# senikm/trpx

Measured on AMD Instinct MI355X. Metric: frames/s (Terse encode + Prolix decode round trip, 512x512 uint16 stack, bit-exact vs CPU ref), higher is better.
Workload: dtype u16

## Files before the change

__graft_entry__.py:

```python
import os
import subprocess
import sys

ROOT = os.path.dirname(os.path.abspath(__file__))
if ROOT not in sys.path:
    sys.path.insert(0, ROOT)


def build() -> None:
    jobs = str(min(8, os.cpu_count() or 1))
    subprocess.check_call(["make", "-s", "-j", jobs, "-C", os.path.join(ROOT, "trpx_amd", "csrc")])
    subprocess.check_call(["make", "-s", "-C", os.path.join(ROOT, "trpx_amd", "csrc"), "force_timeout", "weakparts", "chain_timeout", "denseserial", "densetiny", "segfbgrid", "segwgrounds", "alldense", "noclassify"])
    subprocess.check_call(["make", "-s", "-C", os.path.join(ROOT, "oracle"), "all"])
    if os.path.isdir("/root/reference/include"):
        subprocess.check_call(["make", "-s", "-C", os.path.join(ROOT, "oracle"), "ref"])
    subprocess.check_call(["make", "-s", "-C", os.path.join(ROOT, "trpx_amd", "cli")])
    subprocess.check_call(["make", "-s", "-C", os.path.join(ROOT, "tests", "cpp")])
    subprocess.check_call(["make", "-s", "-C", os.path.join(ROOT, "tests", "cpp"), "-f", "roi_example.mk"])
    subprocess.check_call(["make", "-s", "-C", os.path.join(ROOT, "tests", "cpp"), "-f", "encode_sparse_example.mk"])
    subprocess.check_call(["make", "-s", "-C", os.path.join(ROOT, "tests", "cpp"), "-f", "decode_plan_test.mk"])
    subprocess.check_call([os.path.join(ROOT, "tests", "cpp", "encode_sparse_sanitize")], stdout=subprocess.DEVNULL)
    import tempfile
    with tempfile.TemporaryDirectory() as d:
        subprocess.check_call([os.path.join(ROOT, "tests", "cpp", "host_sanitize"), os.path.join(d, "t.trpx")], stdout=subprocess.DEVNULL)
    import trpx_amd
    from trpx_amd import _lib
    _lib.lib()
# ... 35 lines not shown
```

trpx_amd/csrc/encode_fused.hip:

```cpp
#include <stddef.h>
#include <utility>
#include "codec_common.hpp"
#include "launchers.hpp"
#include "profile.hpp"
#include <stdlib.h>
#include <mutex>
#include <vector>

namespace trpx {

#ifndef TRPX_FUSED_SUB32
#define TRPX_FUSED_SUB32 5
#endif
#ifndef TRPX_FUSED_SUB16
#define TRPX_FUSED_SUB16 4
#endif
template <typename T> constexpr int sub_tiles() { return sizeof(T) <= 2 ? TRPX_FUSED_SUB16 : TRPX_FUSED_SUB32; }
#ifndef TRPX_FUSED_OCC16
#define TRPX_FUSED_OCC16 8
#endif
#ifndef TRPX_FUSED_OCC32
#define TRPX_FUSED_OCC32 4
#endif
template <typename T> constexpr int fused_occupancy() { return sizeof(T) == 1 ? 8 : (sizeof(T) == 2 ? TRPX_FUSED_OCC16 : TRPX_FUSED_OCC32); }
// ... 70 lines not shown
    }
    *result = acc;
    return true;
}

constexpr int kAccShift = 40;
#ifndef TRPX_FUSED_ACC_LINES
#define TRPX_FUSED_ACC_LINES 2
#endif
constexpr uint32_t kAccLines = TRPX_FUSED_ACC_LINES;
__host__ __device__ inline uint32_t fused_acc_lines(uint32_t tiles_per_frame) {
    const uint32_t k = (tiles_per_frame + 31u) / 32u;
    return k < 1u ? 1u : (k > kAccLines ? kAccLines : k);
}
constexpr uint64_t kPrefFlag = 1ull << 63;
__device__ bool lookback_frames(const uint64_t* __restrict__ acc_w, const uint64_t* __restrict__ pref_w, int64_t frame,
                                uint64_t tiles_per_frame, uint64_t* result, uint64_t stride, uint32_t n_acc) {
    const int lane = lane_id();
    uint64_t acc = 0;
    int64_t pos = frame - 1;
    while (pos >= 0) {
        const int64_t my = pos - lane;
        const bool in = my >= 0;
        uint64_t p = in ? 0ull : kPrefFlag, c = 0;
        uint32_t first_p = 64;
        SpinGuard guard;
        uint64_t need = ~0ull;
        bool complete = false;
        for (;;) {
            if (in && !(p & kPrefFlag) && !complete && ((need >> lane) & 1ull)) {
// ... 21 lines not shown
}

template <typename T> struct Raw {
    static constexpr int bits = PixelTraits<T>::bits;
    static constexpr int per = 32 / bits;
    static constexpr int dw = kBlock / per;
};

template <typename T>
__device__ __forceinline__ uint32_t raw_field(const uint32_t (&raw)[Raw<T>::dw], int k) {
    constexpr int per = Raw<T>::per, bits = Raw<T>::bits;
    const uint32_t x = raw[k / per] >> ((k % per) * bits);
    return bits == 32 ? x : x & ((1u << (bits & 31)) - 1u);
}

template <typename T> struct QuadVec;
template <> struct QuadVec<uint8_t>  { typedef uint32_t type; };
template <> struct QuadVec<int8_t>   { typedef uint32_t type; };
template <> struct QuadVec<uint16_t> { typedef uint32_t type __attribute__((ext_vector_type(2))); };
template <> struct QuadVec<int16_t>  { typedef uint32_t type __attribute__((ext_vector_type(2))); };
template <> struct QuadVec<uint32_t> { typedef uint32_t type __attribute__((ext_vector_type(4))); };
template <> struct QuadVec<int32_t>  { typedef uint32_t type __attribute__((ext_vector_type(4))); };

template <typename T>
__device__ __forceinline__ void load_raw_nt(const T* __restrict__ p, uint32_t (&raw)[Raw<T>::dw]) {
    if constexpr (sizeof(T) == 2) {
        typedef uint32_t u4 __attribute__((ext_vector_type(4)));
        typedef uint32_t u2 __attribute__((ext_vector_type(2)));
        u4 lo; u2 hi;
        __builtin_memcpy(&lo, p, 16);
// ... 28 lines not shown
    __builtin_memcpy(&lo, q, 16);
    __builtin_memcpy(&hi, q + 16, 8);
    __builtin_memcpy(&last, q + 24, 2);
    raw[0] = __builtin_amdgcn_alignbit(lo.y, lo.x, 16); raw[1] = __builtin_amdgcn_alignbit(lo.z, lo.y, 16);
    raw[2] = __builtin_amdgcn_alignbit(lo.w, lo.z, 16); raw[3] = __builtin_amdgcn_alignbit(hi.x, lo.w, 16);
    raw[4] = __builtin_amdgcn_alignbit(hi.y, hi.x, 16); raw[5] = __builtin_amdgcn_alignbit((uint32_t)last, hi.y, 16);
}
template <typename T>
__device__ __forceinline__ void load_raw_partial(const T* __restrict__ p, int nb, uint32_t (&raw)[Raw<T>::dw]) {
    using UT = typename PixelTraits<T>::U;
#pragma unroll
    for (int i = 0; i < Raw<T>::dw; ++i) raw[i] = 0;
#pragma unroll
    for (int k = 0; k < kBlock; ++k)
        if (k < nb) raw[k / Raw<T>::per] |= (uint32_t)(UT)p[k] << ((k % Raw<T>::per) * Raw<T>::bits);
}

template <typename T>
__device__ __forceinline__ uint32_t raw_width(const uint32_t (&raw)[Raw<T>::dw]) {
    constexpr int bits = Raw<T>::bits;
    uint32_t m = 0;
    if (!PixelTraits<T>::is_signed) {
#pragma unroll
        for (int i = 0; i < Raw<T>::dw; ++i) m |= raw[i];
        if (bits == 16) m = (m | (m >> 16)) & 0xFFFFu;
        if (bits == 8) { m |= m >> 16; m = (m | (m >> 8)) & 0xFFu; }
    } else if (bits == 32) {
#pragma unroll
        for (int i = 0; i < Raw<T>::dw; ++i) {
            const uint32_t u = raw[i];
// ... 135 lines not shown
    uint64_t* bnd_pos;
    uint64_t* frame_acc;
    uint64_t* frame_pref;
    uint64_t* frame_base;
    uint32_t acc_stride;
    uint32_t n_acc;
    uint64_t* ws_tag;
    uint64_t expect_tag;
    uint64_t* frame_offsets;
    uint32_t* out32;
    uint32_t* status;
    uint8_t* idx_widths;
    uint64_t* idx_group_off;
    uint32_t debug;
    uint64_t* stamps;
};

typedef const char __attribute__((address_space(4)))* karg_ptr;
#define TRPX_KARG(kb, field) (*reinterpret_cast<const decltype(FusedArgs::field) __attribute__((address_space(4)))*>((kb) + 8 + offsetof(FusedArgs, field)))

template <typename T, bool MIS2>
__device__ __forceinline__ void encode_fused_body(const T* __restrict__ pixels, const FusedArgs& a) {
    constexpr int kSub = sub_tiles<T>();
    constexpr int kFusedTileBlocks = kSub * kThreads;
    constexpr int kStage = fused_stage_dwords<T>();
    constexpr int kStage4 = (kStage + 1 + 3) / 4;
    __shared__ __attribute__((aligned(16))) uint32_t s_stage_pad[4 * kStage4];
    uint32_t* const s_stage = s_stage_pad + 1;
    __shared__ uint32_t s_hdr[40];
    __shared__ uint32_t s_wtot[kSub * 4];
    __shared__ uint32_t s_wfl[kSub * 4];
    __shared__ uint64_t s_excl_bits;
    __shared__ uint64_t s_base_bytes;
    __shared__ uint32_t s_abort;
    __shared__ uint32_t s_carry;
    __shared__ uint32_t s_halo;

    const uint32_t tid = threadIdx.x;
#define TRPX_STAMP(slot) do { if ((TRPX_DIAG(a) & 4u) && threadIdx.x == 0) a.stamps[((uint64_t)(blockIdx.z * kGridY + blockIdx.y) * gridDim.x + blockIdx.x) * 8 + (slot)] = __builtin_amdgcn_s_memrealtime(); } while (0)
    TRPX_STAMP(0);
    const int lane = lane_id(), wave = wave_id();
    const FrameGeom g = a.g;
    const uint32_t t = blockIdx.x;
    const uint32_t frame = blockIdx.z * kGridY + blockIdx.y;
    const uint32_t n_frames = a.n_frames, tpf = a.tiles_per_frame;
    asm volatile("" :: "s"(g.n_values), "s"(g.n_blocks), "s"(n_frames), "s"(tpf), "s"(pixels));
    if (frame >= n_frames) return;
    const uint64_t tile = (uint64_t)frame * tpf + t;
    const bool last_tile_of_frame = t + 1 == tpf;
    if (tile == 0 && tid == 0) {
        karg_ptr kb0 = (karg_ptr)__builtin_amdgcn_kernarg_segment_ptr();
        uint64_t* const st64 = reinterpret_cast<uint64_t*>(TRPX_KARG(kb0, status));
#pragma unroll
        for (int i = 0; i < 4; ++i) st_desc(st64 + i, 0ull);
        const uint64_t want = TRPX_KARG(kb0, expect_tag);
        if (want != 0ull && ld_desc(TRPX_KARG(kb0, ws_tag)) != want) atomicMax(&TRPX_KARG(kb0, status)[0], 7u);
        asm volatile("s_waitcnt vmcnt(0)" ::: "memory");
    }
    const T* fp = pixels + (uint64_t)frame * g.n_values;
    const uint32_t b0 = t * kFusedTileBlocks;

    uint32_t v[kSub][Raw<T>::dw];
    uint32_t w[kSub], up[kSub], len[kSub], inc[kSub];
    int nb[kSub];
    const bool has_full = g.n_values >= (uint64_t)kBlock;
    const uint64_t max_first = has_full ? g.n_values - kBlock : 0;
    uint32_t h[Raw<T>::dw];
    [[maybe_unused]] const bool mis2 = MIS2 && ((uintptr_t)fp & 2u) != 0u && frame != 0u;
    if (has_full) {
        bool loaded = false;
        if constexpr (MIS2 && sizeof(T) == 2) {
            if (mis2) {
#pragma unroll
                for (int r = 0; r < kSub; ++r) {
                    const uint64_t first = (uint64_t)(b0 + r * kThreads + tid) * kBlock;
                    load_raw_mis2<T>(fp + (first < max_first ? first : max_first), v[r]);
                }
                loaded = true;
            }
        }
        if (!loaded) {
#pragma unroll
            for (int r = 0; r < kSub; ++r) {
                const uint64_t first = (uint64_t)(b0 + r * kThreads + tid) * kBlock;
                load_raw_nt<T>(fp + (first < max_first ? first : max_first), v[r]);
            }
        }
        if (wave == 0) load_raw_nt<T>(fp + (uint64_t)(b0 ? b0 - 1 : 0) * kBlock, h);
        else {
#pragma unroll
            for (int i = 0; i < Raw<T>::dw; ++i) h[i] = 0u;
        }
    } else {
#pragma unroll
        for (int r = 0; r < kSub; ++r)
#pragma unroll
            for (int i = 0; i < Raw<T>::dw; ++i) v[r][i] = 0u;
#pragma unroll
        for (int i = 0; i < Raw<T>::dw; ++i) h[i] = 0u;
    }
    const uint32_t nb_tail = (uint32_t)(g.n_values - (uint64_t)(g.n_blocks - 1) * kBlock);
#pragma unroll
    for (int r = 0; r < kSub; ++r) {
        const uint32_t b1 = b0 + r * kThreads + tid + 1u;
        nb[r] = b1 < g.n_blocks ? kBlock : (b1 == g.n_blocks ? (int)nb_tail : 0);
    }
    if (tid == 0) s_abort = 0;
    if (tid <= 32u) s_hdr[tid] = header_val(tid, tid + 1u) << (32u - header_len(tid, tid + 1u));
    {
        typedef uint32_t u4 __attribute__((ext_vector_type(4)));
        u4* z = reinterpret_cast<u4*>(s_stage_pad);
#pragma unroll
        for (int i = 0; i < (kStage4 + kThreads - 1) / kThreads; ++i)
            if (i * kThreads + (int)tid < kStage4) z[i * kThreads + tid] = (u4)(0u);
    }
    uint32_t pv[Raw<T>::dw];
#pragma unroll
    for (int i = 0; i < Raw<T>::dw; ++i) pv[i] = 0u;
    if (last_tile_of_frame && g.n_values % kBlock) {
        const uint32_t bp = g.n_blocks - 1;
        if (bp >= b0 && (bp - b0) % kThreads == tid) load_raw_partial<T>(fp + (uint64_t)bp * kBlock, (int)(g.n_values % kBlock), pv);
    }
    TRPX_STAMP(7);
    uint32_t w_part = 0u;
    if (last_tile_of_frame && g.n_values % kBlock) w_part = raw_width<T>(pv);
    if (wave == 0) {
        const uint32_t hw0 = b0 > 0 ? raw_width<T>(h) : 0u;
        if (lane == 0) s_halo = hw0;
    }
    uint32_t wmax = 0;
    uint32_t hlr[kSub];
#pragma unroll
    for (int r = 0; r < kSub; ++r) {
        w[r] = nb[r] == kBlock ? raw_width<T>(v[r]) : (nb[r] ? w_part : 0u);
        wmax = w[r] > wmax ? w[r] : wmax;
        if (a.idx_widths && nb[r]) a.idx_widths[(uint64_t)frame * g.n_blocks + b0 + r * kThreads + tid] = (uint8_t)w[r];
        up[r] = (uint32_t)__builtin_amdgcn_update_dpp(0, (int)w[r], 0x138, 0xf, 0xf, false);
        hlr[r] = header_len(w[r], up[r]);
        len[r] = nb[r] ? (lane ? hlr[r] : 0u) + (uint32_t)nb[r] * w[r] : 0u;
    }
    static_assert(kWave * max_block_bits<T>() < 65536, "packed scan needs 16-bit wave totals");
#pragma unroll
    for (int r = 0; r + 1 < kSub; r += 2) {
        const uint32_t two = wave_inclusive_scan(len[r] | (len[r + 1] << 16));
        inc[r] = two & 0xFFFFu;
        inc[r + 1] = two >> 16;
    }
    if (kSub & 1) inc[kSub - 1] = wave_inclusive_scan(len[kSub - 1]);
    const uint32_t wmax_wave = wave_max(wmax);
#pragma unroll
    for (int r = 0; r < kSub; ++r) {
// ... 25 lines not shown
        const uint32_t hw = h0 | (wprev << 8);
        const int swave = __builtin_amdgcn_readfirstlane(wave);
#pragma unroll
        for (int r = 0; r < kSub; ++r) {
            rb[r] = (uint32_t)__builtin_amdgcn_readlane((int)excl, r * 4);
            const uint32_t pb = (uint32_t)__builtin_amdgcn_readlane((int)excl, r * 4 + swave);
            const uint32_t ph = (uint32_t)__builtin_amdgcn_readlane((int)hw, r * 4 + swave);
            off[r] = pb + (lane ? (ph & 0xFFu) : 0u) + inc[r] - len[r];
            const uint32_t wp_r = lane ? up[r] : ph >> 8;
            const uint32_t hl_r = lane ? hlr[r] : (ph & 0xFFu);
            meta[r] = w[r] | (wp_r << 8) | (hl_r << 16) | (nb[r] == kBlock ? 1u << 24 : 0u) | (nb[r] ? 1u << 25 : 0u);
        }
        rb[kSub] = (uint32_t)__builtin_amdgcn_readlane((int)incl, kSub * 4 - 1);
    }
    const uint32_t tile_total = rb[kSub];

    if (tid == 0 && !(TRPX_DIAG(a) & 1u)) {
        st_desc(a.tile_desc + tile, make_desc(t == 0 ? kStPrefix : kStAgg, tile_total));
        __hip_atomic_fetch_add(a.frame_acc + (uint64_t)frame * a.acc_stride + 16u * (t % a.n_acc), (1ull << kAccShift) | tile_total, __ATOMIC_RELAXED, __HIP_MEMORY_SCOPE_AGENT);
    }
    constexpr int kPhaseRounds = fused_phase_rounds<T>();
    constexpr uint32_t kCapBits = (uint32_t)kPhaseRounds * kThreads * max_block_bits<T>();
    const bool two_phase = tile_total > kCapBits;
    uint64_t p0 = 0, p_end = 0;
    uint64_t img_p0 = 0;
    uint32_t bias = 0;
    bool writable = false;
#ifndef TRPX_ABLATE
#define TRPX_ABLATE 0
#endif
#define TRPX_WSTAMP(slot) do { if ((TRPX_DIAG(a) & 8u) && lane == 0 && tile < 4096) a.stamps[tile * 32 + wave * 8 + (slot)] = __builtin_amdgcn_s_memrealtime(); } while (0)
    auto pack_round = [&](auto rc) {
        constexpr int r = decltype(rc)::value;
        const uint32_t pos = off[r] - bias;
        const uint32_t mr = meta[r];
        const uint32_t hl = (mr >> 16) & 0xFFu;
        const uint32_t wr = mr & 0xFFu;
        const uint32_t hv_top = wr == ((mr >> 8) & 0xFFu) ? 0x80000000u : s_hdr[wr];
        const bool full = (mr >> 24) & 1u;
        if (((mr >> 25) & 1u) && !full && !(TRPX_ABLATE & 2)) {
            const uint64_t hx = (uint64_t)(hv_top >> (32u - hl)) << (pos & 31u);
            atomicOr(&s_stage[pos >> 5], (uint32_t)hx);
            if ((uint32_t)(hx >> 32)) atomicOr(&s_stage[(pos >> 5) + 1], (uint32_t)(hx >> 32));
            if (wr) pack_payload_generic<T>(s_stage, pos + hl, wr, (int)nb_tail, pv);
        }
        uint64_t todo = (TRPX_ABLATE & 1) ? 0ull : __ballot(full);
        while (todo) {
            const int l0 = __builtin_ctzll(todo);
            const uint32_t w0 = (uint32_t)__builtin_amdgcn_readlane((int)wr, l0);
            const bool mine = full && wr == w0;
            uint32_t wd = w0;
            asm volatile("" : "+s"(wd));
#pragma unroll
            for (int i = 0; i < Raw<T>::dw; ++i) asm volatile("" : "+v"(v[r][i]));
            if (mine) PackDispatch<T, 0, PixelTraits<T>::bits>::run(s_stage_pad, pos + hl, hv_top, wd, v[r]);
            todo &= ~__ballot(mine);
        }
        TRPX_WSTAMP(1 + r);
    };
    auto look_back = [&]() {
        if (wave == 0) {
            uint64_t excl = 0;
            bool ok = true;
            if (TRPX_DIAG(a) & 1u) excl = (uint64_t)t * 40000u;
            else if (t != 0) {
                ok = lookback(a.tile_desc, (int64_t)tile, (int64_t)(tile - t), &excl);
                if (ok && lane == 0) st_desc(a.tile_desc + tile, make_desc(kStPrefix, excl + tile_total));
            }
            if (lane == 0) { s_excl_bits = excl; if (!ok) s_abort = 1; }
            TRPX_STAMP(2);
        } else if (wave == 1) {
            uint64_t base = 0;
            bool ok = true;
            if (TRPX_DIAG(a) & 1u) base = (uint64_t)frame * 120000u;
            else if (t == 0) {
                ok = lookback_frames(a.frame_acc, a.frame_pref, (int64_t)frame, a.tiles_per_frame, &base, a.acc_stride, a.n_acc);
                if (ok && lane == 0) st_desc(a.frame_base + (uint64_t)frame * 16, kPrefFlag | base);
            } else {
                uint64_t vb = 0;
                SpinGuard guard;
                for (;;) {
                    vb = ld_desc(a.frame_base + (uint64_t)frame * 16);
                    if (vb & kPrefFlag) break;
                    if (guard.expired()) { ok = false; break; }
                    __builtin_amdgcn_s_sleep(2);
                }
                base = vb & ~kPrefFlag;
            }
            if (lane == 0) { s_base_bytes = base; if (!ok) s_abort = 1; }
        }
    };
    auto place_tile = [&]() -> bool {
        karg_ptr kb = (karg_ptr)__builtin_amdgcn_kernarg_segment_ptr();
        asm volatile("" : "+s"(kb));
        const bool aborted = s_abort != 0;
        const uint64_t excl_bits = s_excl_bits, base_bytes = s_base_bytes;
        const uint64_t frame_size = 1 + (excl_bits + tile_total) / 8;
        if (last_tile_of_frame && tid == 0 && !aborted) {
            st_desc(TRPX_KARG(kb, frame_pref) + (uint64_t)frame * TRPX_KARG(kb, acc_stride), kPrefFlag | (base_bytes + frame_size));
            TRPX_KARG(kb, frame_offsets)[frame + 1] = base_bytes + frame_size;
            if (frame == 0) TRPX_KARG(kb, frame_offsets)[0] = 0;
            if (frame + 1 == TRPX_KARG(kb, n_frames) && align_up(base_bytes + frame_size, 4) > TRPX_KARG(kb, out_capacity))
                atomicMax(&TRPX_KARG(kb, status)[0], 3u);
        }
        if (aborted) {
            if (tid == 0) atomicMax(&TRPX_KARG(kb, status)[0], 7u);
            return false;
        }
        if (TRPX_KARG(kb, idx_group_off) && tid < (uint32_t)kSub && b0 + tid * kThreads < g.n_blocks) {
            uint32_t rbv = 0;
#pragma unroll
            for (int r = 0; r < kSub; ++r) rbv = tid == (uint32_t)r ? rb[r] : rbv;
            TRPX_KARG(kb, idx_group_off)[(uint64_t)frame * g.n_tiles + (uint64_t)t * kSub + tid] = excl_bits + rbv;
        }
        p0 = 8 * base_bytes + excl_bits;
        p_end = last_tile_of_frame ? 8 * (base_bytes + frame_size) : p0 + tile_total;
        writable = align_up((p_end + 7) / 8, 4) <= TRPX_KARG(kb, out_capacity);
        img_p0 = p0;
        return true;
    };
    auto flush = [&](bool first, bool carry_out, uint64_t q_end) {
        karg_ptr kb = (karg_ptr)__builtin_amdgcn_kernarg_segment_ptr();
        asm volatile("" : "+s"(kb));
        uint32_t* const out32 = TRPX_KARG(kb, out32);
        uint64_t* const tail_desc = TRPX_KARG(kb, tail_desc);
        const uint32_t s0 = (uint32_t)(img_p0 & 31), sh = (32u - s0) & 31u;
        const bool head_pending = s0 != 0;
        const uint64_t d_first = img_p0 >> 5, d_last = q_end >> 5;
        const int32_t k_first = head_pending ? -1 : 0;
        const uint32_t n_out = (uint32_t)(d_last - d_first);
        const bool completed_first = d_last > d_first;
        const bool is_last_tile = tile + 1 == (uint64_t)TRPX_KARG(kb, n_frames) * TRPX_KARG(kb, tiles_per_frame);
        if (tid == 0) {
            const int32_t kt = k_first + (int32_t)n_out;
            const uint32_t tail_bits = (q_end & 31) ? __builtin_amdgcn_alignbit(s_stage[kt + 1], s_stage[kt], sh) : 0u;
            if (head_pending) {
// ... 51 lines not shown
        }
    };

    TRPX_WSTAMP(0);
    [&]<int... R>(std::integer_sequence<int, R...>) { (pack_round(std::integral_constant<int, R>{}), ...); }(std::make_integer_sequence<int, kPhaseRounds>{});
    if (two_phase) {
        look_back();
        __syncthreads();
        if (!place_tile()) return;
        flush(true, true, p0 + rb[kPhaseRounds]);
        const uint64_t d_last = (p0 + rb[kPhaseRounds]) >> 5;
        __syncthreads();
        {
            typedef uint32_t u4 __attribute__((ext_vector_type(4)));
            u4* z = reinterpret_cast<u4*>(s_stage_pad);
            for (int i = (int)tid; i < kStage4; i += kThreads) z[i] = (u4)(0u);
        }
        __syncthreads();
        if (tid == 0 && s_carry) atomicOr(&s_stage[0], s_carry);
        img_p0 = 32 * d_last;
        bias = (uint32_t)(img_p0 - p0);
    }
    [&]<int... R>(std::integer_sequence<int, R...>) { (pack_round(std::integral_constant<int, kPhaseRounds + R>{}), ...); }(std::make_integer_sequence<int, kSub - kPhaseRounds>{});
    if (!two_phase) look_back();
    __syncthreads();
    TRPX_STAMP(3);
    if (!two_phase && !place_tile()) return;
    flush(!two_phase, false, p_end);
    TRPX_STAMP(4);
    if ((TRPX_DIAG(a) & 4u) && tid == 0) { uint32_t xcc; asm volatile("s_getreg_b32 %0, hwreg(HW_REG_XCC_ID)" : "=s"(xcc)); a.stamps[tile * 8 + 6] = xcc; }
}

template <typename T>
__global__ __launch_bounds__(kThreads, fused_occupancy<T>()) void k_encode_fused(const T* __restrict__ pixels, FusedArgs a) {
    encode_fused_body<T, false>(pixels, a);
}
template <typename T>
__global__ __launch_bounds__(kThreads, fused_occupancy<T>() - 1) void k_encode_fused_mis2(const T* __restrict__ pixels, FusedArgs a) {
    encode_fused_body<T, true>(pixels, a);
}

__global__ __launch_bounds__(kThreads) void k_stitch(uint64_t* __restrict__ tile_desc, uint64_t* __restrict__ xw, const uint64_t* __restrict__ pos,
                                                     uint64_t n_tiles, uint64_t* __restrict__ frame_words, uint64_t n_frame_words,
                                                     uint64_t* __restrict__ ws_tag, uint64_t tag, uint32_t* __restrict__ out32,
                                                     uint64_t out_capacity, uint32_t* __restrict__ status) {
    __shared__ uint32_t s_max[4];
    const uint64_t b = (uint64_t)blockIdx.x * kThreads + threadIdx.x;
// ... 29 lines not shown
        xw[k] = 0ull;
    }
    if (4 * d + 4 <= out_capacity) out32[d] = acc;
}

template <typename T>
static uint32_t fused_tiles_per_frame(const FrameGeom& g) {
    constexpr uint32_t tb = sub_tiles<T>() * kThreads;
    return (g.n_blocks + tb - 1) / tb;
}

size_t fused_workspace_bytes(const FrameGeom& g, size_t n_frames) {
    const size_t tpf = ((size_t)g.n_blocks + 2 * kThreads - 1) / (2 * kThreads);
    return align_up(8 * (3 * n_frames * tpf + 16 * ((size_t)kAccLines + 1) * n_frames + 1), 256) + 64 * n_frames * tpf;
}

namespace {
struct CleanSig {
    uint32_t elem, tiles_per_frame, n_frames, n_blocks;
    bool operator==(const CleanSig& o) const { return elem == o.elem && tiles_per_frame == o.tiles_per_frame && n_frames == o.n_frames && n_blocks == o.n_blocks; }
};
struct CleanWs { int device; const void* ptr; CleanSig sig; uint64_t tag; };
std::mutex g_clean_mu;
std::vector<CleanWs> g_clean;
uint64_t g_next_tag = 0x5452505800000001ull;
}
void fused_ws_forget(const void* lo, size_t bytes, const void* keep) {
    std::lock_guard<std::mutex> lk(g_clean_mu);
    const char* a = static_cast<const char*>(lo);
    for (size_t i = 0; i < g_clean.size();) {
// ... 13 lines not shown
    a.tile_desc = static_cast<uint64_t*>(ws);
    a.tail_desc = a.tile_desc + tiles;
    a.bnd_pos = a.tail_desc + tiles;
    a.n_acc = fused_acc_lines(a.tiles_per_frame);
    a.acc_stride = 16u * a.n_acc;
    a.frame_acc = a.bnd_pos + tiles;
    a.frame_pref = a.frame_acc + 1;
    a.frame_base = a.frame_acc + (size_t)a.acc_stride * e.n_frames;
    a.frame_offsets = e.frame_offsets;
    a.out32 = reinterpret_cast<uint32_t*>(e.out);
    a.status = e.status;
    a.idx_widths = e.idx_widths;
    a.idx_group_off = e.idx_group_off;
    const size_t frame_words = 16 * ((size_t)a.n_acc + 1) * e.n_frames;
    uint64_t* const frame_words_base = a.frame_acc;
    a.ws_tag = frame_words_base + frame_words;
    a.stamps = reinterpret_cast<uint64_t*>(static_cast<char*>(ws) + align_up(8 * (3 * tiles + frame_words + 1), 256));
#ifdef TRPX_DIAGNOSTICS
    a.debug = getenv("TRPX_FUSED_DEBUG") ? (uint32_t)atoi(getenv("TRPX_FUSED_DEBUG")) : 0u;
#else
    a.debug = 0u;
#endif
    hipStreamCaptureStatus cap = hipStreamCaptureStatusNone;
    if (hipStreamIsCapturing(st, &cap) != hipSuccess) { (void)hipGetLastError(); cap = hipStreamCaptureStatusActive; }
    const bool capturing = cap != hipStreamCaptureStatusNone;
    int device = -1;
    (void)hipGetDevice(&device);
    const CleanSig sig{(uint32_t)sizeof(T), a.tiles_per_frame, e.n_frames, e.geom.n_blocks};
    uint64_t expect = 0, tag = 0;
    if (!capturing) {
// ... 8 lines not shown
    }
    a.expect_tag = expect;
    Profiler& prof = profiler();
    prof.begin();
    prof.mark(st);
    if (expect == 0)
        hipLaunchKernelGGL(k_zero_words<0>, dim3(256), dim3(kThreads), 0, st, static_cast<uint64_t*>(ws),
                           (uint64_t)(3 * tiles + frame_words + (capturing ? 0 : 1)), reinterpret_cast<uint64_t*>(e.status), (uint64_t)4);
    prof.mark(st);
    const dim3 grid(a.tiles_per_frame, e.n_frames < kGridY ? e.n_frames : kGridY, (e.n_frames + kGridY - 1) / kGridY);
    bool mis2 = false;
    if constexpr (sizeof(T) == 2) mis2 = (((uintptr_t)e.pixels & 2u) != 0u || (e.geom.n_values & 1u) != 0u) && e.n_frames > 1u;
    if constexpr (sizeof(T) == 2) {
        if (mis2) hipLaunchKernelGGL((k_encode_fused_mis2<T>), grid, dim3(kThreads), 0, st, static_cast<const T*>(e.pixels), a);
    }
    if (!mis2) hipLaunchKernelGGL((k_encode_fused<T>), grid, dim3(kThreads), 0, st, static_cast<const T*>(e.pixels), a);
    prof.mark(st);
    hipLaunchKernelGGL(k_stitch, dim3((uint32_t)((tiles + kThreads - 1) / kThreads)), dim3(kThreads), 0, st,
                       a.tile_desc, a.tail_desc, static_cast<const uint64_t*>(a.bnd_pos), (uint64_t)tiles, frame_words_base, (uint64_t)frame_words,
                       capturing ? static_cast<uint64_t*>(nullptr) : a.ws_tag, tag, a.out32, (uint64_t)e.out_capacity, a.status);
    prof.mark(st);
    const hipError_t err = hipGetLastError();
    if (err == hipSuccess && !capturing) {
        std::lock_guard<std::mutex> lk(g_clean_mu);
        if (g_clean.size() >= 64) g_clean.erase(g_clean.begin());
        g_clean.push_back(CleanWs{device, ws, sig, tag});
    }
    return err;
}

hipError_t launch_encode_fused(int dtype, const EncodeArgs& e, void* ws, hipStream_t st) {
    return for_pixel_type(dtype, [&]<class T>() { return launch_fused_t<T>(e, ws, st); });
}

}
```

Before: 3.723 million.

## Add persistent ticket-scheduled fused encode kernel that prefetches the next tile

Adds a persistent variant of the fused Terse encoder for 8/16-bit unsigned pixels. A grid sized to resident occupancy draws tiles from sharded atomic ticket counters and issues the pixel loads for its next tile before finishing the current tile's look-back and flush. The aim is to hide global-load latency and avoid block launch and tail overhead across many frames. The partial last block is now derived from already-loaded registers, and the halo load is narrowed to one dword per lane. In exchange it adds ticket atomics, higher register pressure and considerably more complex control flow.

```diff
diff --git a/__graft_entry__.py b/__graft_entry__.py
--- a/__graft_entry__.py
+++ b/__graft_entry__.py
@@ -10,7 +10,7 @@
 def build() -> None:
     jobs = str(min(8, os.cpu_count() or 1))
     subprocess.check_call(["make", "-s", "-j", jobs, "-C", os.path.join(ROOT, "trpx_amd", "csrc")])
-    subprocess.check_call(["make", "-s", "-C", os.path.join(ROOT, "trpx_amd", "csrc"), "force_timeout", "weakparts", "chain_timeout", "denseserial", "densetiny", "segfbgrid", "segwgrounds", "alldense", "noclassify"])
+    subprocess.check_call(["make", "-s", "-C", os.path.join(ROOT, "trpx_amd", "csrc"), "force_timeout", "pipe3", "weakparts", "chain_timeout", "denseserial", "densetiny", "segfbgrid", "segwgrounds", "alldense", "noclassify"])
     subprocess.check_call(["make", "-s", "-C", os.path.join(ROOT, "oracle"), "all"])
     if os.path.isdir("/root/reference/include"):
         subprocess.check_call(["make", "-s", "-C", os.path.join(ROOT, "oracle"), "ref"])
diff --git a/trpx_amd/csrc/encode_fused.hip b/trpx_amd/csrc/encode_fused.hip
--- a/trpx_amd/csrc/encode_fused.hip
+++ b/trpx_amd/csrc/encode_fused.hip
@@ -108,6 +108,10 @@
     return k < 1u ? 1u : (k > kAccLines ? kAccLines : k);
 }
 constexpr uint64_t kPrefFlag = 1ull << 63;
+#ifndef TRPX_FUSED_TICKET_SHARDS
+#define TRPX_FUSED_TICKET_SHARDS 8
+#endif
+constexpr uint32_t kTicketShards = TRPX_FUSED_TICKET_SHARDS;
 __device__ bool lookback_frames(const uint64_t* __restrict__ acc_w, const uint64_t* __restrict__ pref_w, int64_t frame,
                                 uint64_t tiles_per_frame, uint64_t* result, uint64_t stride, uint32_t n_acc) {
     const int lane = lane_id();
@@ -159,6 +163,19 @@
     return bits == 32 ? x : x & ((1u << (bits & 31)) - 1u);
 }
 
+__device__ __forceinline__ uint32_t fresh_lane() {
+    uint32_t l;
+    asm volatile("v_mbcnt_lo_u32_b32 %0, -1, 0\n\tv_mbcnt_hi_u32_b32 %0, -1, %0" : "=v"(l));
+    return l;
+}
+__device__ __forceinline__ auto fresh_zero4() {
+    typedef uint32_t u4 __attribute__((ext_vector_type(4)));
+    u4 z;
+    asm volatile("v_mov_b32 %0, 0" : "=v"(z.x)); asm volatile("v_mov_b32 %0, 0" : "=v"(z.y));
+    asm volatile("v_mov_b32 %0, 0" : "=v"(z.z)); asm volatile("v_mov_b32 %0, 0" : "=v"(z.w));
+    return z;
+}
+
 template <typename T> struct QuadVec;
 template <> struct QuadVec<uint8_t>  { typedef uint32_t type; };
 template <> struct QuadVec<int8_t>   { typedef uint32_t type; };
@@ -217,6 +234,19 @@
 #pragma unroll
     for (int k = 0; k < kBlock; ++k)
         if (k < nb) raw[k / Raw<T>::per] |= (uint32_t)(UT)p[k] << ((k % Raw<T>::per) * Raw<T>::bits);
+}
+
+template <typename T>
+__device__ __forceinline__ void raw_tail(const uint32_t (&src)[Raw<T>::dw], uint32_t sbits, uint32_t (&out)[Raw<T>::dw]) {
+    const uint32_t ds = sbits >> 5, bs = sbits & 31u;
+#pragma unroll
+    for (int i = 0; i < Raw<T>::dw; ++i) out[i] = 0u;
+#pragma unroll
+    for (int d = 0; d < Raw<T>::dw; ++d)
+        if (ds == (uint32_t)d) {
+#pragma unroll
+            for (int i = 0; i + d < Raw<T>::dw; ++i) out[i] = __builtin_amdgcn_alignbit(i + d + 1 < Raw<T>::dw ? src[i + d + 1] : 0u, src[i + d], bs);
+        }
 }
 
 template <typename T>
@@ -382,13 +412,17 @@
     uint64_t* idx_group_off;
     uint32_t debug;
     uint64_t* stamps;
+    uint64_t* tickets;
+    uint32_t n_shards;
+    uint32_t n_tiles;
 };
 
 typedef const char __attribute__((address_space(4)))* karg_ptr;
 #define TRPX_KARG(kb, field) (*reinterpret_cast<const decltype(FusedArgs::field) __attribute__((address_space(4)))*>((kb) + 8 + offsetof(FusedArgs, field)))
 
-template <typename T, bool MIS2>
+template <typename T, bool MIS2, bool PIPE = false>
 __device__ __forceinline__ void encode_fused_body(const T* __restrict__ pixels, const FusedArgs& a) {
+    static_assert(!(PIPE && MIS2) && !(PIPE && sizeof(T) > 2), "the pipelined path: aligned 8/16-bit pixels");
     constexpr int kSub = sub_tiles<T>();
     constexpr int kFusedTileBlocks = kSub * kThreads;
     constexpr int kStage = fused_stage_dwords<T>();
@@ -404,18 +438,114 @@
     __shared__ uint32_t s_carry;
     __shared__ uint32_t s_halo;
 
-    const uint32_t tid = threadIdx.x;
-#define TRPX_STAMP(slot) do { if ((TRPX_DIAG(a) & 4u) && threadIdx.x == 0) a.stamps[((uint64_t)(blockIdx.z * kGridY + blockIdx.y) * gridDim.x + blockIdx.x) * 8 + (slot)] = __builtin_amdgcn_s_memrealtime(); } while (0)
-    TRPX_STAMP(0);
-    const int lane = lane_id(), wave = wave_id();
-    const FrameGeom g = a.g;
-    const uint32_t t = blockIdx.x;
-    const uint32_t frame = blockIdx.z * kGridY + blockIdx.y;
+    const uint32_t tid_k = threadIdx.x;
+#define TRPX_STAMP_AT(tile_, slot) do { if ((TRPX_DIAG(a) & 4u) && threadIdx.x == 0) a.stamps[(uint64_t)(tile_) * 8 + (slot)] = __builtin_amdgcn_s_memrealtime(); } while (0)
+#define TRPX_STAMP(slot) TRPX_STAMP_AT(tile, slot)
+    const int lane_k = lane_id(), wave_k = wave_id();
+    const FrameGeom g_k = a.g;
     const uint32_t n_frames = a.n_frames, tpf = a.tiles_per_frame;
-    asm volatile("" :: "s"(g.n_values), "s"(g.n_blocks), "s"(n_frames), "s"(tpf), "s"(pixels));
-    if (frame >= n_frames) return;
+    uint32_t t, frame;
+    [[maybe_unused]] uint32_t next_tile = 0;
+    [[maybe_unused]] __shared__ uint32_t s_ticket0, s_ticket;
+    [[maybe_unused]] uint32_t drawn = 0;
+    constexpr uint32_t kNoTicket = 0xFFFFFFFFu;
+    if constexpr (PIPE) {
+        const uint32_t ns = a.n_shards, shard = blockIdx.x % ns;
+        if (tid_k == 0) s_ticket0 = __hip_atomic_fetch_add(reinterpret_cast<uint32_t*>(a.tickets + 16u * shard), 1u, __ATOMIC_RELAXED, __HIP_MEMORY_SCOPE_AGENT);
+        __syncthreads();
+        const uint32_t cur = (uint32_t)__builtin_amdgcn_readfirstlane((int)s_ticket0) * ns + shard;
+        if (cur >= a.n_tiles) return;
+        frame = cur / tpf;
+        t = cur - frame * tpf;
+    } else {
+        t = blockIdx.x;
+        frame = blockIdx.z * kGridY + blockIdx.y;
+        asm volatile("" :: "s"(g_k.n_values), "s"(g_k.n_blocks), "s"(n_frames), "s"(tpf), "s"(pixels));
+        if (frame >= n_frames) return;
+    }
+    uint32_t v[kSub][Raw<T>::dw];
+    uint32_t h[Raw<T>::dw];
+    uint32_t pv[Raw<T>::dw];
+    auto issue_loads = [&](const FrameGeom& g, uint32_t frame_, uint32_t t_, uint32_t tid, int wave) {
+        const bool has_full = g.n_values >= (uint64_t)kBlock;
+        const uint64_t max_first = has_full ? g.n_values - kBlock : 0;
+        const T* fp = pixels + (uint64_t)frame_ * g.n_values;
+        const uint32_t b0 = t_ * kFusedTileBlocks;
+        [[maybe_unused]] const bool mis2 = MIS2 && ((uintptr_t)fp & 2u) != 0u && frame_ != 0u;
+        if (has_full) {
+            bool loaded = false;
+            if constexpr (MIS2 && sizeof(T) == 2) {
+                if (mis2) {
+#pragma unroll
+                    for (int r = 0; r < kSub; ++r) {
+                        const uint64_t first = (uint64_t)(b0 + r * kThreads + tid) * kBlock;
+                        load_raw_mis2<T>(fp + (first < max_first ? first : max_first), v[r]);
+                    }
+                    loaded = true;
+                }
+            }
+            if (!loaded) {
+#pragma unroll
+                for (int r = 0; r < kSub; ++r) {
+                    const uint64_t first = (uint64_t)(b0 + r * kThreads + tid) * kBlock;
+                    load_raw_nt<T>(fp + (first < max_first ? first : max_first), v[r]);
+                }
+            }
+            if constexpr (PIPE) {
+                h[0] = 0u;
+                if (wave == 0 && (tid & 63u) < (uint32_t)Raw<T>::dw) __builtin_memcpy(&h[0], reinterpret_cast<const char*>(fp + (uint64_t)(b0 ? b0 - 1 : 0) * kBlock) + 4u * tid, 4);
+            } else if (wave == 0) load_raw_nt<T>(fp + (uint64_t)(b0 ? b0 - 1 : 0) * kBlock, h);
+            else {
+#pragma unroll
+                for (int i = 0; i < Raw<T>::dw; ++i) h[i] = 0u;
+            }
+        } else {
+#pragma unroll
+            for (int r = 0; r < kSub; ++r)
+#pragma unroll
+                for (int i = 0; i < Raw<T>::dw; ++i) v[r][i] = 0u;
+#pragma unroll
+            for (int i = 0; i < Raw<T>::dw; ++i) h[i] = 0u;
+            if constexpr (PIPE) {
+                if (tid == 0 && g.n_values) load_raw_partial<T>(fp, (int)g.n_values, v[0]);
+            }
+        }
+        if constexpr (!PIPE) {
+#pragma unroll
+            for (int i = 0; i < Raw<T>::dw; ++i) pv[i] = 0u;
+            if (t_ + 1 == tpf && g.n_values % kBlock) {
+                const uint32_t bp = g.n_blocks - 1;
+                if (bp >= b0 && (bp - b0) % kThreads == tid) load_raw_partial<T>(fp + (uint64_t)bp * kBlock, (int)(g.n_values % kBlock), pv);
+            }
+        }
+    };
+    issue_loads(g_k, frame, t, tid_k, wave_k);
+    if constexpr (PIPE) {
+        if (tid_k == 3 * kWave) {
+            uint32_t* counter = reinterpret_cast<uint32_t*>(a.tickets + 16u * (blockIdx.x % a.n_shards));
+            asm volatile("" : "+v"(counter));
+            drawn = __hip_atomic_fetch_add(counter, 1u, __ATOMIC_RELAXED, __HIP_MEMORY_SCOPE_AGENT);
+        }
+    }
+    [[maybe_unused]] bool first_round = true;
+    karg_ptr kbl = (karg_ptr)__builtin_amdgcn_kernarg_segment_ptr();
+#define TRPX_A(field) (PIPE ? TRPX_KARG(kbl, field) : a.field)
+#define TRPX_A_HERE() do { if constexpr (PIPE) asm volatile("" : "+s"(kbl)); } while (0)
+  for (;;) {
+    TRPX_A_HERE();
+    FrameGeom g = g_k;
+    if constexpr (PIPE) asm volatile("" : "+s"(g.n_values), "+s"(g.n_blocks));
+    const bool has_full = g.n_values >= (uint64_t)kBlock;
+    uint32_t tid = tid_k;
+    if constexpr (PIPE) {
+        tid = fresh_lane() + 64u * (uint32_t)wave_k;
+    }
+    const int lane = PIPE ? (int)(tid & 63u) : lane_k;
+    const int wave = wave_k;
+    if constexpr (PIPE) { if (tid == 3 * kWave) s_ticket = drawn; }
     const uint64_t tile = (uint64_t)frame * tpf + t;
     const bool last_tile_of_frame = t + 1 == tpf;
+    TRPX_STAMP(0);
     if (tile == 0 && tid == 0) {
         karg_ptr kb0 = (karg_ptr)__builtin_amdgcn_kernarg_segment_ptr();
         uint64_t* const st64 = reinterpret_cast<uint64_t*>(TRPX_KARG(kb0, status));
@@ -425,48 +555,9 @@
         if (want != 0ull && ld_desc(TRPX_KARG(kb0, ws_tag)) != want) atomicMax(&TRPX_KARG(kb0, status)[0], 7u);
         asm volatile("s_waitcnt vmcnt(0)" ::: "memory");
     }
-    const T* fp = pixels + (uint64_t)frame * g.n_values;
     const uint32_t b0 = t * kFusedTileBlocks;
-
-    uint32_t v[kSub][Raw<T>::dw];
     uint32_t w[kSub], up[kSub], len[kSub], inc[kSub];
     int nb[kSub];
-    const bool has_full = g.n_values >= (uint64_t)kBlock;
-    const uint64_t max_first = has_full ? g.n_values - kBlock : 0;
-    uint32_t h[Raw<T>::dw];
-    [[maybe_unused]] const bool mis2 = MIS2 && ((uintptr_t)fp & 2u) != 0u && frame != 0u;
-    if (has_full) {
-        bool loaded = false;
-        if constexpr (MIS2 && sizeof(T) == 2) {
-            if (mis2) {
-#pragma unroll
-                for (int r = 0; r < kSub; ++r) {
-                    const uint64_t first = (uint64_t)(b0 + r * kThreads + tid) * kBlock;
-                    load_raw_mis2<T>(fp + (first < max_first ? first : max_first), v[r]);
-                }
-                loaded = true;
-            }
-        }
-        if (!loaded) {
-#pragma unroll
-            for (int r = 0; r < kSub; ++r) {
-                const uint64_t first = (uint64_t)(b0 + r * kThreads + tid) * kBlock;
-                load_raw_nt<T>(fp + (first < max_first ? first : max_first), v[r]);
-            }
-        }
-        if (wave == 0) load_raw_nt<T>(fp + (uint64_t)(b0 ? b0 - 1 : 0) * kBlock, h);
-        else {
-#pragma unroll
-            for (int i = 0; i < Raw<T>::dw; ++i) h[i] = 0u;
-        }
-    } else {
-#pragma unroll
-        for (int r = 0; r < kSub; ++r)
-#pragma unroll
-            for (int i = 0; i < Raw<T>::dw; ++i) v[r][i] = 0u;
-#pragma unroll
-        for (int i = 0; i < Raw<T>::dw; ++i) h[i] = 0u;
-    }
     const uint32_t nb_tail = (uint32_t)(g.n_values - (uint64_t)(g.n_blocks - 1) * kBlock);
 #pragma unroll
     for (int r = 0; r < kSub; ++r) {
@@ -478,22 +569,35 @@
     {
         typedef uint32_t u4 __attribute__((ext_vector_type(4)));
         u4* z = reinterpret_cast<u4*>(s_stage_pad);
+        u4 zero4 = (u4)(0u);
+        if constexpr (PIPE) zero4 = fresh_zero4();
 #pragma unroll
         for (int i = 0; i < (kStage4 + kThreads - 1) / kThreads; ++i)
-            if (i * kThreads + (int)tid < kStage4) z[i * kThreads + tid] = (u4)(0u);
-    }
-    uint32_t pv[Raw<T>::dw];
-#pragma unroll
-    for (int i = 0; i < Raw<T>::dw; ++i) pv[i] = 0u;
+            if (i * kThreads + (int)tid < kStage4) z[i * kThreads + tid] = zero4;
+    }
+    if (!PIPE || first_round) TRPX_STAMP(7);
+    uint32_t w_part = 0u;
+    [[maybe_unused]] const uint32_t part_sbits = has_full ? (kBlock - (uint32_t)(g.n_values % kBlock)) * Raw<T>::bits : 0u;
     if (last_tile_of_frame && g.n_values % kBlock) {
-        const uint32_t bp = g.n_blocks - 1;
-        if (bp >= b0 && (bp - b0) % kThreads == tid) load_raw_partial<T>(fp + (uint64_t)bp * kBlock, (int)(g.n_values % kBlock), pv);
-    }
-    TRPX_STAMP(7);
-    uint32_t w_part = 0u;
-    if (last_tile_of_frame && g.n_values % kBlock) w_part = raw_width<T>(pv);
+        if constexpr (PIPE) {
+            const uint32_t rp = (g.n_blocks - 1 - b0) / kThreads;
+#pragma unroll
+            for (int r = 0; r < kSub; ++r)
+                if (rp == (uint32_t)r) {
+                    uint32_t part[Raw<T>::dw];
+                    raw_tail<T>(v[r], part_sbits, part);
+                    w_part = raw_width<T>(part);
+                }
+        } else w_part = raw_width<T>(pv);
+    }
     if (wave == 0) {
-        const uint32_t hw0 = b0 > 0 ? raw_width<T>(h) : 0u;
+        uint32_t hw0;
+        if constexpr (PIPE) {
+            uint32_t piece[Raw<T>::dw];
+#pragma unroll
+            for (int i = 0; i < Raw<T>::dw; ++i) piece[i] = i == 0 ? h[0] : 0u;
+            hw0 = b0 > 0 ? wave_max(raw_width<T>(piece)) : 0u;
+        } else hw0 = b0 > 0 ? raw_width<T>(h) : 0u;
         if (lane == 0) s_halo = hw0;
     }
     uint32_t wmax = 0;
@@ -502,7 +606,7 @@
     for (int r = 0; r < kSub; ++r) {
         w[r] = nb[r] == kBlock ? raw_width<T>(v[r]) : (nb[r] ? w_part : 0u);
         wmax = w[r] > wmax ? w[r] : wmax;
-        if (a.idx_widths && nb[r]) a.idx_widths[(uint64_t)frame * g.n_blocks + b0 + r * kThreads + tid] = (uint8_t)w[r];
+        if (TRPX_A(idx_widths) && nb[r]) TRPX_A(idx_widths)[(uint64_t)frame * g.n_blocks + b0 + r * kThreads + tid] = (uint8_t)w[r];
         up[r] = (uint32_t)__builtin_amdgcn_update_dpp(0, (int)w[r], 0x138, 0xf, 0xf, false);
         hlr[r] = header_len(w[r], up[r]);
         len[r] = nb[r] ? (lane ? hlr[r] : 0u) + (uint32_t)nb[r] * w[r] : 0u;
@@ -558,10 +662,14 @@
         rb[kSub] = (uint32_t)__builtin_amdgcn_readlane((int)incl, kSub * 4 - 1);
     }
     const uint32_t tile_total = rb[kSub];
+    if constexpr (PIPE) {
+        const uint32_t tk = (uint32_t)__builtin_amdgcn_readfirstlane((int)s_ticket);
+        next_tile = tk == kNoTicket ? kNoTicket : tk * TRPX_A(n_shards) + blockIdx.x % TRPX_A(n_shards);
+    }
 
     if (tid == 0 && !(TRPX_DIAG(a) & 1u)) {
-        st_desc(a.tile_desc + tile, make_desc(t == 0 ? kStPrefix : kStAgg, tile_total));
-        __hip_atomic_fetch_add(a.frame_acc + (uint64_t)frame * a.acc_stride + 16u * (t % a.n_acc), (1ull << kAccShift) | tile_total, __ATOMIC_RELAXED, __HIP_MEMORY_SCOPE_AGENT);
+        st_desc(TRPX_A(tile_desc) + tile, make_desc(t == 0 ? kStPrefix : kStAgg, tile_total));
+        __hip_atomic_fetch_add(TRPX_A(frame_acc) + (uint64_t)frame * TRPX_A(acc_stride) + 16u * (t % TRPX_A(n_acc)), (1ull << kAccShift) | tile_total, __ATOMIC_RELAXED, __HIP_MEMORY_SCOPE_AGENT);
     }
     constexpr int kPhaseRounds = fused_phase_rounds<T>();
     constexpr uint32_t kCapBits = (uint32_t)kPhaseRounds * kThreads * max_block_bits<T>();
@@ -586,7 +694,11 @@
             const uint64_t hx = (uint64_t)(hv_top >> (32u - hl)) << (pos & 31u);
             atomicOr(&s_stage[pos >> 5], (uint32_t)hx);
             if ((uint32_t)(hx >> 32)) atomicOr(&s_stage[(pos >> 5) + 1], (uint32_t)(hx >> 32));
-            if (wr) pack_payload_generic<T>(s_stage, pos + hl, wr, (int)nb_tail, pv);
+            if constexpr (PIPE) {
+                uint32_t part[Raw<T>::dw];
+                raw_tail<T>(v[r], part_sbits, part);
+                if (wr) pack_payload_generic<T>(s_stage, pos + hl, wr, (int)nb_tail, part);
+            } else if (wr) pack_payload_generic<T>(s_stage, pos + hl, wr, (int)nb_tail, pv);
         }
         uint64_t todo = (TRPX_ABLATE & 1) ? 0ull : __ballot(full);
         while (todo) {
@@ -603,13 +715,14 @@
         TRPX_WSTAMP(1 + r);
     };
     auto look_back = [&]() {
+        TRPX_A_HERE();
         if (wave == 0) {
             uint64_t excl = 0;
             bool ok = true;
             if (TRPX_DIAG(a) & 1u) excl = (uint64_t)t * 40000u;
             else if (t != 0) {
-                ok = lookback(a.tile_desc, (int64_t)tile, (int64_t)(tile - t), &excl);
-                if (ok && lane == 0) st_desc(a.tile_desc + tile, make_desc(kStPrefix, excl + tile_total));
+                ok = lookback(TRPX_A(tile_desc), (int64_t)tile, (int64_t)(tile - t), &excl);
+                if (ok && lane == 0) st_desc(TRPX_A(tile_desc) + tile, make_desc(kStPrefix, excl + tile_total));
             }
             if (lane == 0) { s_excl_bits = excl; if (!ok) s_abort = 1; }
             TRPX_STAMP(2);
@@ -618,13 +731,13 @@
             bool ok = true;
             if (TRPX_DIAG(a) & 1u) base = (uint64_t)frame * 120000u;
             else if (t == 0) {
-                ok = lookback_frames(a.frame_acc, a.frame_pref, (int64_t)frame, a.tiles_per_frame, &base, a.acc_stride, a.n_acc);
-                if (ok && lane == 0) st_desc(a.frame_base + (uint64_t)frame * 16, kPrefFlag | base);
+                ok = lookback_frames(TRPX_A(frame_acc), TRPX_A(frame_pref), (int64_t)frame, TRPX_A(tiles_per_frame), &base, TRPX_A(acc_stride), TRPX_A(n_acc));
+                if (ok && lane == 0) st_desc(TRPX_A(frame_base) + (uint64_t)frame * 16, kPrefFlag | base);
             } else {
                 uint64_t vb = 0;
                 SpinGuard guard;
                 for (;;) {
-                    vb = ld_desc(a.frame_base + (uint64_t)frame * 16);
+                    vb = ld_desc(TRPX_A(frame_base) + (uint64_t)frame * 16);
                     if (vb & kPrefFlag) break;
                     if (guard.expired()) { ok = false; break; }
                     __builtin_amdgcn_s_sleep(2);
@@ -638,7 +751,11 @@
         karg_ptr kb = (karg_ptr)__builtin_amdgcn_kernarg_segment_ptr();
         asm volatile("" : "+s"(kb));
         const bool aborted = s_abort != 0;
-        const uint64_t excl_bits = s_excl_bits, base_bytes = s_base_bytes;
+        uint64_t excl_bits = s_excl_bits, base_bytes = s_base_bytes;
+        if constexpr (PIPE) {
+            excl_bits = (uint64_t)(uint32_t)__builtin_amdgcn_readfirstlane((int)excl_bits) | (uint64_t)(uint32_t)__builtin_amdgcn_readfirstlane((int)(excl_bits >> 32)) << 32;
+            base_bytes = (uint64_t)(uint32_t)__builtin_amdgcn_readfirstlane((int)base_bytes) | (uint64_t)(uint32_t)__builtin_amdgcn_readfirstlane((int)(base_bytes >> 32)) << 32;
+        }
         const uint64_t frame_size = 1 + (excl_bits + tile_total) / 8;
         if (last_tile_of_frame && tid == 0 && !aborted) {
             st_desc(TRPX_KARG(kb, frame_pref) + (uint64_t)frame * TRPX_KARG(kb, acc_stride), kPrefFlag | (base_bytes + frame_size));
@@ -663,7 +780,8 @@
         img_p0 = p0;
         return true;
     };
-    auto flush = [&](bool first, bool carry_out, uint64_t q_end) {
+    auto flush = [&, tid_round = tid](bool first, bool carry_out, uint64_t q_end) {
+        const uint32_t tid = PIPE ? fresh_lane() + 64u * (uint32_t)wave_k : tid_round;
         karg_ptr kb = (karg_ptr)__builtin_amdgcn_kernarg_segment_ptr();
         asm volatile("" : "+s"(kb));
         uint32_t* const out32 = TRPX_KARG(kb, out32);
@@ -745,7 +863,9 @@
         {
             typedef uint32_t u4 __attribute__((ext_vector_type(4)));
             u4* z = reinterpret_cast<u4*>(s_stage_pad);
-            for (int i = (int)tid; i < kStage4; i += kThreads) z[i] = (u4)(0u);
+            u4 zero4 = (u4)(0u);
+            if constexpr (PIPE) zero4 = fresh_zero4();
+            for (int i = (int)tid; i < kStage4; i += kThreads) z[i] = zero4;
         }
         __syncthreads();
         if (tid == 0 && s_carry) atomicOr(&s_stage[0], s_carry);
@@ -754,14 +874,68 @@
     }
     [&]<int... R>(std::integer_sequence<int, R...>) { (pack_round(std::integral_constant<int, kPhaseRounds + R>{}), ...); }(std::make_integer_sequence<int, kSub - kPhaseRounds>{});
     if (!two_phase) look_back();
+    if constexpr (PIPE) {
+        TRPX_A_HERE();
+        if (wave == 3 && fresh_lane() == 0u) {
+            drawn = kNoTicket;
+            if (next_tile < TRPX_A(n_tiles)) {
+                uint32_t* counter = reinterpret_cast<uint32_t*>(TRPX_A(tickets) + 16u * (blockIdx.x % TRPX_A(n_shards)));
+                asm volatile("" : "+v"(counter));
+                drawn = __hip_atomic_fetch_add(counter, 1u, __ATOMIC_RELAXED, __HIP_MEMORY_SCOPE_AGENT);
+            }
+        }
+        if (next_tile < TRPX_A(n_tiles)) {
+            const uint32_t nf = next_tile / tpf;
+            issue_loads(g, nf, next_tile - nf * tpf, fresh_lane() + 64u * (uint32_t)wave_k, wave);
+            TRPX_STAMP_AT(next_tile, 7);
+        }
+    }
     __syncthreads();
     TRPX_STAMP(3);
     if (!two_phase && !place_tile()) return;
     flush(!two_phase, false, p_end);
     TRPX_STAMP(4);
-    if ((TRPX_DIAG(a) & 4u) && tid == 0) { uint32_t xcc; asm volatile("s_getreg_b32 %0, hwreg(HW_REG_XCC_ID)" : "=s"(xcc)); a.stamps[tile * 8 + 6] = xcc; }
-}
-
+    if ((TRPX_DIAG(a) & 4u) && tid == 0) { uint32_t xcc; asm volatile("s_getreg_b32 %0, hwreg(HW_REG_XCC_ID)" : "=s"(xcc)); a.stamps[tile * 8 + 6] = xcc | (PIPE ? (uint64_t)blockIdx.x << 8 : 0ull); }
+    if constexpr (!PIPE) return;
+    else {
+        TRPX_A_HERE();
+        if (next_tile >= TRPX_A(n_tiles)) return;
+        frame = next_tile / tpf;
+        t = next_tile - frame * tpf;
+        first_round = false;
+        __syncthreads();
+    }
+  }
+}
+
+template <typename T> constexpr bool fused_has_pipe() { return sizeof(T) == 1 || (sizeof(T) == 2 && !PixelTraits<T>::is_signed); }
+hipError_t launch_fused_pipe(int dtype, uint32_t grid, hipStream_t st, const void* pixels, const FusedArgs& a);
+uint32_t fused_pipe_per_cu(int dtype);
+
+#ifdef TRPX_FUSED_PIPE_TU
+template <typename T>
+__global__ __launch_bounds__(kThreads, fused_occupancy<T>()) void k_encode_fused_pipe(const T* __restrict__ pixels, FusedArgs a) {
+    encode_fused_body<T, false, true>(pixels, a);
+}
+hipError_t launch_fused_pipe(int dtype, uint32_t grid, hipStream_t st, const void* pixels, const FusedArgs& a) {
+    return for_pixel_type(dtype, [&]<class T>() {
+        if constexpr (fused_has_pipe<T>()) {
+            hipLaunchKernelGGL((k_encode_fused_pipe<T>), dim3(grid), dim3(kThreads), 0, st, static_cast<const T*>(pixels), a);
+            return hipSuccess;
+        } else return hipErrorInvalidValue;
+    });
+}
+uint32_t fused_pipe_per_cu(int dtype) {
+    int per_cu = 0;
+    (void)for_pixel_type(dtype, [&]<class T>() {
+        if constexpr (fused_has_pipe<T>()) {
+            if (hipOccupancyMaxActiveBlocksPerMultiprocessor(&per_cu, k_encode_fused_pipe<T>, kThreads, 0) != hipSuccess) { (void)hipGetLastError(); per_cu = 0; }
+        }
+        return hipSuccess;
+    });
+    return per_cu > 0 ? (uint32_t)per_cu : 0u;
+}
+#else
 template <typename T>
 __global__ __launch_bounds__(kThreads, fused_occupancy<T>()) void k_encode_fused(const T* __restrict__ pixels, FusedArgs a) {
     encode_fused_body<T, false>(pixels, a);
@@ -821,6 +995,32 @@
     const size_t tpf = ((size_t)g.n_blocks + 2 * kThreads - 1) / (2 * kThreads);
     return align_up(8 * (3 * n_frames * tpf + 16 * ((size_t)kAccLines + 1) * n_frames + 1), 256) + 64 * n_frames * tpf;
 }
+
+template <typename T>
+static uint32_t fused_pipe_grid() {
+#if defined(TRPX_FUSED_NO_PIPE)
+    return 0u;
+#elif defined(TRPX_FUSED_PIPE_GRID)
+    return fused_has_pipe<T>() ? TRPX_FUSED_PIPE_GRID : 0u;
+#else
+    if constexpr (!fused_has_pipe<T>()) return 0u;
+    else {
+        static thread_local int cached_dev = -1;
+        static thread_local uint32_t cached = 0;
+        int dev = 0;
+        if (hipGetDevice(&dev) != hipSuccess) return 0u;
+        if (dev == cached_dev) return cached;
+        int cus = 0;
+        const uint32_t per_cu = fused_pipe_per_cu(PixelTraits<T>::dtype);
+        if (hipDeviceGetAttribute(&cus, hipDeviceAttributeMultiprocessorCount, dev) != hipSuccess || cus < 1) cus = 0;
+        (void)hipGetLastError();
+        cached = per_cu * (uint32_t)cus;
+        cached_dev = dev;
+        return cached;
+    }
+#endif
+}
+static thread_local int g_last_route = -1;
 
 namespace {
 struct CleanSig {
@@ -864,6 +1064,7 @@
     a.idx_group_off = e.idx_group_off;
     const size_t frame_words = 16 * ((size_t)a.n_acc + 1) * e.n_frames;
     uint64_t* const frame_words_base = a.frame_acc;
+    a.tickets = a.frame_base + 8;
     a.ws_tag = frame_words_base + frame_words;
     a.stamps = reinterpret_cast<uint64_t*>(static_cast<char*>(ws) + align_up(8 * (3 * tiles + frame_words + 1), 256));
 #ifdef TRPX_DIAGNOSTICS
@@ -902,7 +1103,14 @@
     if constexpr (sizeof(T) == 2) {
         if (mis2) hipLaunchKernelGGL((k_encode_fused_mis2<T>), grid, dim3(kThreads), 0, st, static_cast<const T*>(e.pixels), a);
     }
-    if (!mis2) hipLaunchKernelGGL((k_encode_fused<T>), grid, dim3(kThreads), 0, st, static_cast<const T*>(e.pixels), a);
+    const uint32_t pipe_grid = mis2 || tiles >= (1ull << 31) ? 0u : fused_pipe_grid<T>();
+    const bool pipe = pipe_grid != 0u && tiles > pipe_grid;
+    a.n_tiles = (uint32_t)(tiles < (1ull << 31) ? tiles : 0u);
+    a.n_shards = pipe_grid < kTicketShards ? (pipe_grid ? pipe_grid : 1u) : kTicketShards;
+    if (a.n_shards > e.n_frames) a.n_shards = e.n_frames;
+    if (pipe) (void)launch_fused_pipe(PixelTraits<T>::dtype, pipe_grid, st, e.pixels, a);
+    if (!mis2 && !pipe) hipLaunchKernelGGL((k_encode_fused<T>), grid, dim3(kThreads), 0, st, static_cast<const T*>(e.pixels), a);
+    g_last_route = pipe ? 1 : (mis2 ? 2 : 0);
     prof.mark(st);
     hipLaunchKernelGGL(k_stitch, dim3((uint32_t)((tiles + kThreads - 1) / kThreads)), dim3(kThreads), 0, st,
                        a.tile_desc, a.tail_desc, static_cast<const uint64_t*>(a.bnd_pos), (uint64_t)tiles, frame_words_base, (uint64_t)frame_words,
@@ -920,5 +1128,18 @@
 hipError_t launch_encode_fused(int dtype, const EncodeArgs& e, void* ws, hipStream_t st) {
     return for_pixel_type(dtype, [&]<class T>() { return launch_fused_t<T>(e, ws, st); });
 }
-
-}
+uint32_t fused_pipe_grid_of(int dtype) {
+    uint32_t n = 0;
+    (void)for_pixel_type(dtype, [&]<class T>() { n = fused_pipe_grid<T>(); return hipSuccess; });
+    return n;
+}
+
+#endif
+}
+
+#ifndef TRPX_FUSED_PIPE_TU
+extern "C" {
+__attribute__((visibility("default"))) unsigned trpx_debug_encode_pipe_grid(int dtype) { return trpx::fused_pipe_grid_of(dtype); }
+__attribute__((visibility("default"))) int trpx_debug_encode_last_route(void) { return trpx::g_last_route; }
+}
+#endif
diff --git a/trpx_amd/csrc/encode_fused_pipe.hip b/trpx_amd/csrc/encode_fused_pipe.hip
--- /dev/null
+++ b/trpx_amd/csrc/encode_fused_pipe.hip
@@ -0,0 +1,2 @@
+#define TRPX_FUSED_PIPE_TU
+#include "encode_fused.hip"
```

Measured after the change: 2.640 million. 0.709x the previous value.
